# Rocco9999/2048_Q-Learning

Hardware: AMD Instinct MI355X
Metric: env_steps_per_sec (higher is better)
Workload: dtype u8

## Files before the change

2048_q-learning_amd/csrc/q2048_core.hpp:

```cpp
#pragma once
#include <stdint.h>
#include <math.h>

#if defined(__HIPCC__)
#define Q_HD __host__ __device__ __forceinline__
#else
#define Q_HD inline
#endif

#include "q2048_luts.inc"

namespace q2048 {

constexpr uint32_t kStreamStep = 0u, kStreamReset = 1u, kStreamOver = 2u;

struct Draws { uint32_t x0, x1, x2, x3; };

#ifndef Q2048_PHILOX_ROUNDS
#define Q2048_PHILOX_ROUNDS 10
#endif
Q_HD void philox_round(uint32_t& c0, uint32_t& c1, uint32_t& c2, uint32_t& c3, uint32_t k0, uint32_t k1) {
  const uint64_t p0 = (uint64_t)0xD2511F53u * c0;
  const uint64_t p1 = (uint64_t)0xCD9E8D57u * c2;
  const uint32_t n0 = (uint32_t)(p1 >> 32) ^ c1 ^ k0;
// ... 507 lines not shown

Q_HD uint64_t summary_fp(uint64_t hash) { return ((hash >> 48) & 0xffffull) | 1ull; }
struct SummaryHits { uint32_t ev, empty; };
Q_HD SummaryHits summary_decode(uint64_t word, uint64_t fp, uint32_t off) {
  uint32_t e = 0u, m = 0u;
#pragma unroll
  for (uint32_t r = 0; r < 4u; ++r) {
    const uint64_t f = (word >> (16u * r)) & 0xffffull;
    e |= (uint32_t)(f == 0ull) << r;
    m |= (uint32_t)(f == fp) << r;
  }
  return SummaryHits{(((e | m) | ((e | m) << 4)) >> (off & 3u)) & 15u, e};
}
Q_HD bool summary_pop(SummaryHits& h, uint32_t off, uint32_t& r, bool& absent) {
  if (h.ev == 0u) return false;
  r = (off + (uint32_t)__builtin_ctz(h.ev)) & 3u;
  absent = ((h.empty >> r) & 1u) != 0u;
  h.ev &= h.ev - 1u;
  return true;
}

Q_HD int argmax4(float q0, float q1, float q2, float q3) {
  int b = 0;
  float m = q0;
  if (q1 > m) { m = q1; b = 1; }
  if (q2 > m) { m = q2; b = 2; }
  if (q3 > m) { m = q3; b = 3; }
  return b;
}
Q_HD float max4(float q0, float q1, float q2, float q3) { return fmaxf(fmaxf(q0, q1), fmaxf(q2, q3)); }

Q_HD int eps_greedy(double eps, uint32_t x_eps, uint32_t x_act, float q0, float q1, float q2,
                    float q3, bool& explored) {
  explored = draw_uniform(x_eps) < eps;
  return explored ? draw_action(x_act) : argmax4(q0, q1, q2, q3);
}

Q_HD uint64_t eps_threshold(double eps) {
  if (!(eps > 0.0)) return 0ull;
  if (eps >= 1.0) return 1ull << 32;
  return (uint64_t)ceil(eps * 4294967296.0);
}
Q_HD bool draw_below(uint32_t x, uint64_t threshold) {
  return (threshold >> 32) != 0ull || x < (uint32_t)threshold;
}
Q_HD int eps_greedy_at(uint64_t threshold, uint32_t x_eps, uint32_t x_act, float q0, float q1, float q2,
                       float q3, bool& explored) {
  explored = draw_below(x_eps, threshold);
  return explored ? draw_action(x_act) : argmax4(q0, q1, q2, q3);
}

template <class BoardT>
Q_HD uint32_t legal_mask(const BoardT& b) {
  uint32_t m = 0;
#pragma unroll
  for (int a = 0; a < 4; ++a) {
    BoardT t = b;
    uint32_t score;
    m |= (uint32_t)move(t, a, score) << a;
  }
  return m;
}
Q_HD int play_action(uint32_t legal, float q0, float q1, float q2, float q3, uint64_t threshold, uint32_t x_eps,
                     uint32_t x_act, bool& explored) {
  legal &= 15u;
  const uint32_t n_legal = popc(legal);
  explored = n_legal != 0u && draw_below(x_eps, threshold);
  if (explored) {
    uint32_t k = draw_index(x_act, n_legal), m = legal;
#pragma unroll
    for (int j = 0; j < 3; ++j) { const bool drop = k != 0u; m &= drop ? m - 1u : m; k -= drop ? 1u : 0u; }
    return __builtin_ctz(m);
  }
  int best = 0;
  float top = 0.f;
  bool have = false;
  if (legal & 1u) { top = q0; have = true; }
  if ((legal & 2u) && (!have || q1 > top)) { top = q1; best = 1; have = true; }
  if ((legal & 4u) && (!have || q2 > top)) { top = q2; best = 2; have = true; }
  if ((legal & 8u) && (!have || q3 > top)) { top = q3; best = 3; }
  return best;
}

#if defined(__clang__)
#define Q2048_NO_CONTRACT _Pragma("clang fp contract(off)")
#else
#define Q2048_NO_CONTRACT
#endif
Q_HD double td_target(float reward, float max_q_next, bool done, double gamma) {
  Q2048_NO_CONTRACT
  const double bootstrap = gamma * (double)max_q_next;
  return (double)reward + bootstrap * (done ? 0.0 : 1.0);
}
Q_HD double td_fold(double q, double target, double lr) {
  Q2048_NO_CONTRACT
  const double step = lr * (target - q);
  return q + step;
}
Q_HD float td_value(float q_sa, float reward, float max_q_next, bool done, double lr,
                    double gamma) {
  return (float)td_fold((double)q_sa, td_target(reward, max_q_next, done, gamma), lr);
}

constexpr int kFoldMean = 0, kFoldMeanTrained = 1, kFoldSum = 2, kFoldMaxAbs = 3;
Q_HD void key_images(uint64_t k, uint64_t img[8]) {
  const uint64_t t = key_transpose(k), hk = key_flip_h(k), ht = key_flip_h(t);
  img[0] = k; img[1] = key_flip_v(t); img[2] = key_flip_v(hk); img[3] = ht;
  img[4] = hk; img[5] = t; img[6] = key_flip_v(k); img[7] = key_flip_v(ht);
}
Q_HD float fold_inv(uint32_t k) {
  return k == 1u ? 1.0f : k == 2u ? 0.5f : k == 3u ? (float)(1.0 / 3.0) : k == 4u ? 0.25f : k == 5u ? (float)(1.0 / 5.0)
       : k == 6u ? (float)(1.0 / 6.0) : k == 7u ? (float)(1.0 / 7.0) : 0.125f;
}
template <int FOLD>
Q_HD void fold_step(float& acc, uint32_t& n, float x) {
  Q2048_NO_CONTRACT
  if (FOLD == kFoldMeanTrained && x == 0.0f) return;
  if (n == 0u) acc = x;
  else if (FOLD == kFoldMaxAbs) acc = fabsf(x) > fabsf(acc) ? x : acc;
  else acc = acc + x;
  n += 1u;
}
template <int FOLD>
Q_HD float fold_finish(float acc, uint32_t n) {
  Q2048_NO_CONTRACT
  if (FOLD == kFoldMean || FOLD == kFoldMeanTrained) {
    const float inv = fold_inv(n);
    return n == 0u ? 0.0f : acc * inv;
  }
  return acc;
}
template <int FOLD, class Find>
Q_HD bool fold_orbit(uint64_t m, const float q[4], const Find& find, uint64_t& canon, float r[4]) {
  canon = canonical_key(m).key;
  uint64_t img[8];
  key_images(canon, img);
  float acc[4] = {0.0f, 0.0f, 0.0f, 0.0f};
  uint32_t n[4] = {0u, 0u, 0u, 0u};
  bool leader = false;
#pragma unroll
  for (int h = 0; h < 8; ++h) {
    bool repeat = false;
#pragma unroll
    for (int j = 0; j < h; ++j) repeat |= img[j] == img[h];
    if (repeat) continue;
    float v[4];
    if (img[h] == m) {
      leader = true;
      v[0] = q[0]; v[1] = q[1]; v[2] = q[2]; v[3] = q[3];
    } else {
      if (!find(img[h], v)) continue;
      if (!leader) return false;
    }
    const uint32_t g = canonical_key(img[h]).g;
#pragma unroll
    for (int a = 0; a < 4; ++a) {
      const int at = sym_action(g, a);
#pragma unroll
      for (int b = 0; b < 4; ++b)
        if (at == b) fold_step<FOLD>(acc[b], n[b], v[a]);
    }
  }
#pragma unroll
  for (int b = 0; b < 4; ++b) r[b] = fold_finish<FOLD>(acc[b], n[b]);
  return true;
}
// ... 37 lines not shown
```

2048_q-learning_amd/csrc/q2048_core5.hpp:

```cpp
#pragma once
#include "q2048_core.hpp"

namespace q2048 {

struct Board5 { uint32_t r[5]; };

constexpr uint32_t k5One = 0x01041041u;
constexpr uint32_t k5Low = k5One * 31u;
constexpr uint32_t k5High = k5One << 5;
constexpr uint32_t k5All = k5One * 63u;

Q_HD uint32_t nz5(uint32_t x) { return (x + k5Low) & k5High; }
Q_HD uint32_t z5(uint32_t x) { return ~(x + k5Low) & k5High; }
Q_HD uint32_t fill5(uint32_t m) { return m - (m >> 5); }
Q_HD uint32_t field5(uint32_t w, int c) { return (w >> (6 * c)) & 63u; }

Q_HD bool operator==(const Board5& a, const Board5& b) {
  uint32_t d = 0;
#pragma unroll
  for (int i = 0; i < 5; ++i) d |= a.r[i] ^ b.r[i];
  return d == 0;
}
Q_HD void clear(Board5& b) {
#pragma unroll
// ... 118 lines not shown
  for (int i = 1; i < 5; ++i) {
    const bool ge = k >= before[i];
    x = ge ? g[i] : x; base = ge ? before[i] : base; row += ge ? 1u : 0u;
  }
  const uint32_t skip = k - base;
#pragma unroll
  for (uint32_t j = 0; j < 4u; ++j) x = skip > j ? x & (x - 1u) : x;
  x &= 0u - x;
  const uint32_t w = x >> (draw_is_four(draw_val) ? 4u : 5u);
#pragma unroll
  for (int i = 0; i < 5; ++i) b.r[i] |= row == (uint32_t)i ? w : 0u;
  return n;
}
Q_HD void spawn(Board5& b, uint32_t draw_pos, uint32_t draw_val) { spawn_counted(b, true, draw_pos, draw_val); }

Q_HD bool game_over(const Board5& b) {
  uint32_t live = 0;
#pragma unroll
  for (int i = 0; i < 5; ++i) {
    live |= z5(b.r[i]);
    live |= z5(b.r[i] ^ (b.r[i] >> 6)) & (k5High >> 6);
    if (i < 4) live |= z5(b.r[i] ^ b.r[i + 1]);
  }
  return live == 0u;
}

Q_HD bool equal_neighbours_on_full(const Board5& b) {
  uint32_t acc = k5High;
#pragma unroll
  for (int i = 0; i < 5; ++i) {
    acc &= (b.r[i] ^ (b.r[i] >> 6)) + k5Low;
    if (i < 4) acc &= (b.r[i] ^ b.r[i + 1]) + k5Low;
  }
  return (acc & k5High) != k5High;
}

Q_HD bool spawn_then_over(Board5& b, bool valid, uint32_t draw_pos, uint32_t draw_val) {
  const uint32_t n = spawn_counted(b, valid, draw_pos, draw_val);
  const uint32_t left = n - ((valid && n != 0u) ? 1u : 0u);
  return left == 0u && !equal_neighbours_on_full(b);
}

Q_HD uint32_t fieldmax5(uint32_t a, uint32_t b) {
  const uint32_t m = fill5(((a | k5High) - b) & k5High);
  return bsel(m, a, b);
}
Q_HD uint32_t max_log2(const Board5& b) {
  uint32_t x = fieldmax5(fieldmax5(b.r[0], b.r[1]), fieldmax5(fieldmax5(b.r[2], b.r[3]), b.r[4]));
  uint32_t m = field5(x, 0);
#pragma unroll
  for (int c = 1; c < 5; ++c) { const uint32_t f = field5(x, c); m = f > m ? f : m; }
  return m;
}

struct Key5 { uint64_t k0, k1; };
Q_HD uint32_t pack_row5(uint32_t r) {
  return (r & 31u) | ((r >> 1) & (31u << 5)) | ((r >> 2) & (31u << 10)) | ((r >> 3) & (31u << 15)) |
         ((r >> 4) & (31u << 20));
}
Q_HD Key5 pack_key(const Board5& b) {
  const uint64_t p0 = pack_row5(b.r[0]), p1 = pack_row5(b.r[1]), p2 = pack_row5(b.r[2]),
                 p3 = pack_row5(b.r[3]), p4 = pack_row5(b.r[4]);
  return Key5{(p0 | (p1 << 25) | ((p2 & 0x1fffull) << 50)) | (1ull << 63),
              ((p2 >> 13) | (p3 << 12) | (p4 << 37)) | (1ull << 63)};
}
Q_HD uint32_t unpack_row5(uint32_t p) {
  return (p & 31u) | ((p & (31u << 5)) << 1) | ((p & (31u << 10)) << 2) | ((p & (31u << 15)) << 3) |
         ((p & (31u << 20)) << 4);
}
Q_HD Board5 unpack_key(const Key5& k) {
  const uint64_t a = k.k0 & ~(1ull << 63), c = k.k1 & ~(1ull << 63);
  Board5 b;
  b.r[0] = unpack_row5((uint32_t)(a & 0x1ffffffull));
  b.r[1] = unpack_row5((uint32_t)((a >> 25) & 0x1ffffffull));
  b.r[2] = unpack_row5((uint32_t)(((a >> 50) & 0x1fffull) | ((c & 0xfffull) << 13)));
  b.r[3] = unpack_row5((uint32_t)((c >> 12) & 0x1ffffffull));
  b.r[4] = unpack_row5((uint32_t)((c >> 37) & 0x1ffffffull));
  return b;
}

template <int N> struct Geo;
template <> struct Geo<4> {
  using BoardT = Board;
  struct Key { uint64_t k0; };
};
template <> struct Geo<5> {
  using BoardT = Board5;
  struct Key { uint64_t k0, k1; };
};
Q_HD bool key_eq(const Geo<4>::Key& a, const Geo<4>::Key& b) { return a.k0 == b.k0; }
Q_HD bool key_eq(const Geo<5>::Key& a, const Geo<5>::Key& b) { return a.k0 == b.k0 && a.k1 == b.k1; }
Q_HD uint64_t key_hash(const Geo<4>::Key& k) { return mix64(k.k0); }
Q_HD uint64_t key_hash(const Geo<5>::Key& k) { return mix64(k.k0 ^ (k.k1 * 0x9E3779B97F4A7C15ull)); }
template <class Key>
Q_HD uint64_t key_home(const Key& k, uint64_t mask) { return key_hash(k) & mask; }

template <class F>
Q_HD Geo<4>::Key state_key(const Board& b, uint64_t salt, const F& overflow) {
  bool ov;
  const uint64_t k = pack_key(b, ov) ^ salt;
  if (ov) overflow();
  return Geo<4>::Key{k != 0u ? k : 1u};
}
template <class F>
Q_HD Geo<5>::Key state_key(const Board5& b, uint64_t salt, const F&) {
  const Key5 k = pack_key(b);
  return Geo<5>::Key{k.k0 ^ (salt & 0x7fffffffffffffffull), k.k1 ^ (mix64(salt) & 0x3fffffffffffffffull)};
}
template <bool SYM, class BoardT, class F>
Q_HD auto state_key_as(const BoardT& b, uint64_t salt, uint32_t& g, const F& overflow) {
  if constexpr (SYM) {
    bool ov;
    const Canon c = canonical_key(pack_key(b, ov));
    if (ov) overflow();
    g = c.g;
    const uint64_t k = c.key ^ salt;
    return Geo<4>::Key{k != 0u ? k : 1u};
  } else {
    g = 0u;
    return state_key(b, salt, overflow);
  }
}

Q_HD Board5 board5_from_bytes(const uint8_t* p) {
  Board5 b;
#pragma unroll
  for (int i = 0; i < 5; ++i) {
    uint32_t w = 0;
#pragma unroll
    for (int c = 0; c < 5; ++c) w |= ((uint32_t)p[5 * i + c] & 31u) << (6 * c);
    b.r[i] = w;
  }
  return b;
}
Q_HD void board5_to_bytes(const Board5& b, uint8_t* p) {
#pragma unroll
  for (int i = 0; i < 5; ++i)
#pragma unroll
    for (int c = 0; c < 5; ++c) p[5 * i + c] = (uint8_t)(field5(b.r[i], c) & 31u);
}

}
```

2048_q-learning_amd/csrc/q2048_host.cpp:

```cpp
#include <algorithm>
#include <chrono>
#include <cstddef>
#include <cstdint>
#include <cstdlib>
#include <cstring>
#include <thread>
#include <unordered_map>
#include <vector>

#include "q2048_abi.hpp"
#include "q2048_core5.hpp"

namespace {
using namespace q2048;
using u64 = unsigned long long;

constexpr int kMaxAwait = 1 << 20;

static_assert(sizeof(q2048_aux) == 16 && sizeof(q2048_slot) == 32 && sizeof(q2048_episode) == 48, "ABI layout");
static_assert(sizeof(Aux) == sizeof(q2048_aux), "core/ABI aux mismatch");

inline void load_board(const uint8_t* boards, int64_t i, Board& b) { std::memcpy(&b, boards + 16 * i, 16); }
inline void load_board(const uint8_t* boards, int64_t i, Board5& b) { b = board5_from_bytes(boards + 25 * i); }
inline void store_board(uint8_t* boards, int64_t i, const Board& b) { std::memcpy(boards + 16 * i, &b, 16); }
inline void store_board(uint8_t* boards, int64_t i, const Board5& b) { board5_to_bytes(b, boards + 25 * i); }
inline Aux ld_aux(const q2048_aux* aux, int64_t i) {
  Words4 w;
  std::memcpy(&w, aux + i, 16);
  return words_to_aux(w);
}
inline void st_aux(q2048_aux* aux, int64_t i, const Aux& a) {
  const Words4 w = aux_to_words(a);
  std::memcpy(aux + i, &w, 16);
}
inline void status_or(uint32_t* status, uint32_t bits) { __atomic_fetch_or(status, bits, __ATOMIC_RELAXED); }

template <bool SYM, class BoardT>
inline auto state_key_as(const BoardT& b, u64 salt, uint32_t* status, uint32_t& g) {
  return q2048::state_key_as<SYM>(b, salt, g, [status] { status_or(status, Q2048_STATUS_TILE_OVERFLOW); });
}
template <class BoardT>
inline auto state_key(const BoardT& b, u64 salt, uint32_t* status) {
  uint32_t g;
  return state_key_as<false>(b, salt, status, g);
}
template <int N>
inline typename Geo<N>::Key state_key_sym(bool sym, const typename Geo<N>::BoardT& b, u64 salt, uint32_t* status, uint32_t& g) {
  if constexpr (N == 4) { if (sym) return state_key_as<true>(b, salt, status, g); }
  return state_key_as<false>(b, salt, status, g);
}

inline u64 ld_u64(const uint64_t* p) { return __atomic_load_n(p, __ATOMIC_ACQUIRE); }
inline float ld_f32(const float* p) {
  const uint32_t u = __atomic_load_n(reinterpret_cast<const uint32_t*>(p), __ATOMIC_RELAXED);
  return bits_f32(u);
}
inline void st_f32(float* p, float v) { __atomic_store_n(reinterpret_cast<uint32_t*>(p), f32_bits(v), __ATOMIC_RELAXED); }
inline Row ld_row(const q2048_slot* s) { return Row{ld_f32(&s->q[0]), ld_f32(&s->q[1]), ld_f32(&s->q[2]), ld_f32(&s->q[3])}; }

unsigned long long g_claim_timeouts = 0;
inline u64 await_second(const q2048_slot* s) {
  for (int spin = 0; spin < kMaxAwait; ++spin) {
    const u64 hi = ld_u64(&s->reserved);
    if (hi != 0ull) return hi;
    if ((spin & 1023) == 1023) std::this_thread::yield();
  }
  for (const auto give_up = std::chrono::steady_clock::now() + std::chrono::seconds(2); std::chrono::steady_clock::now() < give_up;) {
    std::this_thread::sleep_for(std::chrono::microseconds(50));
    const u64 hi = ld_u64(&s->reserved);
    if (hi != 0ull) return hi;
  }
  __atomic_fetch_add(&g_claim_timeouts, 1ull, __ATOMIC_RELAXED);
  return 0ull;
}
inline bool slot_is(const q2048_slot*, const Geo<4>::Key&) { return true; }
inline bool slot_is(const q2048_slot* s, const Geo<5>::Key& key) {
  u64 hi = ld_u64(&s->reserved);
  if (hi == 0ull) hi = await_second(s);
  return hi == key.k1;
}
inline void publish(q2048_slot*, const Geo<4>::Key&) {}
inline void publish(q2048_slot* s, const Geo<5>::Key& key) { __atomic_store_n(&s->reserved, key.k1, __ATOMIC_RELEASE); }

template <class Key>
inline int64_t probe_find(const q2048_slot* table, u64 mask, const Key& key, Row& row, uint32_t maxp = kRolloutProbe) {
  const Seq sq = seq_of(key_hash(key), mask);
  row = Row{0.f, 0.f, 0.f, 0.f};
  for (uint32_t p = 0, lim = probe_limit(mask, maxp); p < lim; ++p) {
    const u64 i = seq_slot(sq, p);
    const u64 k = ld_u64(&table[i].key);
    if (k == 0ull) return ~(int64_t)i;
    if (k == key.k0 && slot_is(&table[i], key)) { row = ld_row(&table[i]); return (int64_t)i; }
  }
  return kNoSlot;
}
inline int64_t probe_find_summary(const q2048_slot* table, const uint64_t* side, u64 mask, const Geo<5>::Key& key, Row& row,
                                  uint32_t maxp = kRolloutProbe) {
  const u64 hash = key_hash(key);
  const Seq sq = seq_of(hash, mask);
  const u64 fp = summary_fp(hash);
  row = Row{0.f, 0.f, 0.f, 0.f};
  for (uint32_t p = 0, lim = probe_limit(mask, maxp); p < lim; p += 4u) {
    const u64 line = (sq.line0 + (u64)(p >> 2)) & sq.lmask;
    SummaryHits hits = summary_decode(ld_u64(&side[line]), fp, sq.off);
    uint32_t r;
    bool absent;
    while (summary_pop(hits, sq.off, r, absent)) {
      const u64 i = (line << 2) | (u64)r;
      if (absent) return ~(int64_t)i;
      if (ld_u64(&table[i].key) == key.k0 && ld_u64(&table[i].reserved) == key.k1) { row = ld_row(&table[i]); return (int64_t)i; }
    }
  }
  return kNoSlot;
}
inline int64_t probe_find_summary(const q2048_slot* table, const uint64_t*, u64 mask, const Geo<4>::Key& key, Row& row) {
  return probe_find(table, mask, key, row);
}
template <class Key>
inline int64_t probe_insert(q2048_slot* table, u64 mask, const Key& key, u64 start, bool& inserted,
                            uint32_t maxp = kRolloutProbe) {
  const Seq sq = seq_of(key_hash(key), mask);
  inserted = false;
  u64 i = start & mask;
  for (uint32_t p = seq_pos(sq, i), lim = probe_limit(mask, maxp); p < lim; i = seq_slot(sq, ++p)) {
    uint64_t k = ld_u64(&table[i].key);
    if (k == 0ull) {
      uint64_t expect = 0ull;
      if (__atomic_compare_exchange_n(&table[i].key, &expect, (uint64_t)key.k0, false, __ATOMIC_ACQ_REL, __ATOMIC_ACQUIRE)) {
        publish(&table[i], key);
        inserted = true;
// ... 268 lines not shown
  if (!boards || !actions || !status) return Q2048_ERR_NULL;
  if (!aligned16(boards) || !aligned16(row_cache)) return Q2048_ERR_ALIGN;
  if (!(eps >= 0.0 && eps <= 1.0)) return Q2048_ERR_RANGE;
  if (B == 0) return Q2048_OK;
  const u64 mask = (1ull << cap_log2) - 1ull;
  if (n == 4) q_choose_impl_n<4>(table, mask, boards, B, eps, seed, env_id0, ctr, flags, actions, status, draw_eps, draw_act, row_cache);
  else q_choose_impl_n<5>(table, mask, boards, B, eps, seed, env_id0, ctr, flags, actions, status, draw_eps, draw_act, row_cache);
  return Q2048_OK;
}

template <int N>
void q_update_impl_n(q2048_slot* table, u64 mask, const uint8_t* s, const uint8_t* actions, const float* reward,
                     const uint8_t* s2, const uint8_t* done, int64_t B, double lr, double gamma, uint64_t env_id0,
                     uint32_t flags, int64_t* stats_i, uint32_t* status, void* cache) {
  const int T = threads_for(B);
  std::vector<Stats> parts((size_t)T);
  Stats* sp = parts.data();
  const bool cas = (flags & Q2048_FLAG_TD_CAS) != 0, create = (flags & Q2048_FLAG_NO_NEW_ROWS) == 0;
  const int used = parallel_ranges(B, [=](int64_t lo, int64_t hi, int t) {
    Stats& st = sp[t];
    TdCounters tdc;
    for (int64_t i = lo; i < hi; ++i) {
      const int act = actions[i];
      if (act > 3) { status_or(status, Q2048_STATUS_BAD_ACTION); continue; }
      typename Geo<N>::BoardT b_s, b_n;
      load_board(s, i, b_s);
      load_board(s2, i, b_n);
      const u64 salt = (flags & Q2048_FLAG_INDEPENDENT) ? lane_salt(env_id0 + (uint64_t)i) : 0ull;
      const auto key_s = state_key(b_s, salt, status);
      const auto key_n = state_key(b_n, salt, status);
      Row rs, rn;
      bool ins_s = false, ins_n = false;
      int64_t slot = kNoSlot;
      if (!cache_get<N>(cache, i, table, mask, key_s, rs, slot, !create)) slot = find_or_create(table, mask, key_s, rs, ins_s, create);
      rn = rs;
      const bool same = key_eq(key_n, key_s);
      int64_t slot_n = slot;
      if (!same) slot_n = find_or_create(table, mask, key_n, rn, ins_n, create);
      st.i[Q2048_ST_INSERTS] += (uint64_t)ins_s + (uint64_t)ins_n;
      const float max_next = max4(rn.q0, rn.q1, rn.q2, rn.q3);
      if (slot >= 0) {
        const float nq = td_update(&table[slot], act, row_get(rs, act), reward[i], max_next, done[i] != 0, lr, gamma, cas, tdc);
        if (same) row_set(rn, act, nq);
      } else {
        st.i[Q2048_ST_DROPS] += 1;
        if (create) status_or(status, Q2048_STATUS_TABLE_FULL);
        else if (same) row_set(rn, act, td_value(row_get(rs, act), reward[i], max_next, done[i] != 0, lr, gamma));
      }
      cache_put<N>(cache, i, table, mask, key_n, rn, slot_n, !create);
    }
    st.i[Q2048_ST_CAS_RETRY] += tdc.retries;
    st.i[Q2048_ST_CAS_FALLBACK] += tdc.fallbacks;
  });
  stats_merge(parts, used, stats_i, nullptr);
}

template <int N>
void q_lookup_impl_n(const q2048_slot* table, u64 mask, const uint8_t* boards, int64_t B, uint64_t env_id0,
                     uint32_t flags, float* q_out, uint8_t* found, uint32_t* status) {
  const bool sym = (flags & Q2048_FLAG_SYMMETRIC) != 0;
  parallel_ranges(B, [=](int64_t lo, int64_t hi, int) {
    for (int64_t i = lo; i < hi; ++i) {
      typename Geo<N>::BoardT b;
      load_board(boards, i, b);
      const uint64_t id = (flags & Q2048_FLAG_SINGLE_ENV) ? env_id0 : env_id0 + (uint64_t)i;
      const u64 salt = (flags & Q2048_FLAG_INDEPENDENT) ? lane_salt(id) : 0ull;
      Row r;
      uint32_t g;
      const int64_t slot = probe_find(table, mask, state_key_sym<N>(sym, b, salt, status, g), r, kMaxProbe);
      if (sym) r = row_env(r, g);
      q_out[4 * i] = r.q0; q_out[4 * i + 1] = r.q1; q_out[4 * i + 2] = r.q2; q_out[4 * i + 3] = r.q3;
      if (found != nullptr) found[i] = slot >= 0;
    }
  });
}

constexpr int kGroup = 16;
template <int N>
void fused_rollout_n(uint8_t* boards, q2048_aux* aux, q2048_slot* table, u64 mask, int64_t B, int steps, double eps,
                     double lr, double gamma, uint64_t seed, uint64_t env_id0, uint32_t ctr0, uint32_t flags,
                     int64_t* stats_i, double* stats_f, uint32_t* status, q2048_episode* log, int64_t log_cap,
                     uint64_t* log_count, void* cache, const uint64_t* side) {
  using BoardT = typename Geo<N>::BoardT;
  using Key = typename Geo<N>::Key;
  struct Lane {
    BoardT b; Aux a; Key key_s, key_n; Row q; int64_t slot_s; u64 salt; uint64_t id; double reward_sum;
    StepOut o; int act; bool explored, same; DrawPrep prep;
    uint32_t g_s, g_n;
  };
  const uint64_t eps_t = eps_threshold(eps);
  const ImageLuts lut{&g_lut_image};
  const int env = env_bits(flags);
  const bool play_only = (flags & Q2048_FLAG_PLAY_ONLY) != 0, no_learn = (flags & Q2048_FLAG_NO_LEARN) != 0;
  const bool learns = !play_only && !no_learn, frozen = (flags & Q2048_FLAG_NO_NEW_ROWS) != 0;
  const bool creates = learns && !frozen, cas = (flags & Q2048_FLAG_TD_CAS) != 0;
  const bool sym = N == 4 && !play_only && (flags & Q2048_FLAG_SYMMETRIC) != 0;
  const bool summary = N == 5 && learns && frozen && (flags & Q2048_FLAG_LINE_SUMMARY) != 0 && side != nullptr;
  const int T = threads_for(B);
  std::vector<Stats> parts((size_t)T);
  Stats* sp = parts.data();
  const int used = parallel_ranges(B, [=](int64_t lo, int64_t hi, int tid) {
    auto find = [=](const Key& key, Row& row) {
      return summary ? probe_find_summary(table, side, mask, key, row) : probe_find(table, mask, key, row);
    };
    Stats& st = sp[tid];
    TdCounters tdc;
    bool any_drop = false;
    Lane lane[kGroup];
    for (int64_t g0 = lo; g0 < hi; g0 += kGroup) {
      const int n = (int)(hi - g0 < kGroup ? hi - g0 : kGroup);
      for (int l = 0; l < n; ++l) {
        Lane& L = lane[l];
        const int64_t i = g0 + l;
        L.id = env_id0 + (uint64_t)i;
        L.salt = (flags & Q2048_FLAG_INDEPENDENT) ? lane_salt(L.id) : 0ull;
        load_board(boards, i, L.b);
        L.a = ld_aux(aux, i);
        L.key_s = state_key_sym<N>(sym, L.b, L.salt, status, L.g_s);
        L.q = Row{0.f, 0.f, 0.f, 0.f};
        L.slot_s = play_only ? kNoSlot : find(L.key_s, L.q);
        if (frozen && learns && L.slot_s < 0) visit_get<N>(cache, i, table, mask, L.key_s, L.q);
        L.reward_sum = 0.0;
        L.prep = draws_prepare(seed, L.id, kStreamStep);
      }
      for (int t = 0; t < steps; ++t) {
        for (int l = 0; l < n; ++l) {
          Lane& L = lane[l];
          const Draws x = draws_at(L.prep, ctr0 + (uint32_t)t);
          Draws y{0u, 0u, 0u, 0u};
          if (env & kEnvDqn) y = draws(seed, L.id, ctr0 + (uint32_t)t, kStreamOver);
          const Row qe = sym ? row_env(L.q, L.g_s) : L.q;
          L.act = eps_greedy_at(eps_t, x.x0, x.x1, qe.q0, qe.q1, qe.q2, qe.q3, L.explored);
          L.o = env_step_any(env, L.b, L.a, L.act, x.x2, x.x3, y.x0, y.x1, lut);
          L.key_n = state_key_sym<N>(sym, L.b, L.salt, status, L.g_n);
          L.same = key_eq(L.key_n, L.key_s);
          if (!L.same && !play_only) __builtin_prefetch(&table[key_hash(L.key_n) & mask], 1, 1);
        }
        for (int l = 0; l < n; ++l) {
          Lane& L = lane[l];
          const StepOut& o = L.o;
          const int act = sym ? sym_action(L.g_s, L.act) : L.act;
          bool ins_s = false, ins_n = false;
          if (L.slot_s < 0 && L.slot_s != kNoSlot && creates) L.slot_s = probe_insert(table, mask, L.key_s, (u64)~L.slot_s, ins_s);
          Row qn = L.q;
          int64_t slot_n = L.slot_s;
          if (!L.same) {
            if (play_only) { qn = Row{0.f, 0.f, 0.f, 0.f}; slot_n = kNoSlot; }
            else if (creates) slot_n = find_or_create(table, mask, L.key_n, qn, ins_n);
            else slot_n = find(L.key_n, qn);
          }
          const float max_next = max4(qn.q0, qn.q1, qn.q2, qn.q3);
          const bool updated = L.slot_s >= 0;
          float nq = 0.f;
          if (updated) {
            if (no_learn) nq = td_value(row_get(L.q, act), o.reward, max_next, o.done != 0, lr, gamma);
            else nq = td_update(&table[L.slot_s], act, row_get(L.q, act), o.reward, max_next, o.done != 0, lr, gamma, cas, tdc);
          } else if (frozen && learns) {
            nq = td_value(row_get(L.q, act), o.reward, max_next, o.done != 0, lr, gamma);
          }
          st.i[Q2048_ST_VALID] += o.valid != 0;
          st.i[Q2048_ST_EXPLORE] += L.explored;
          st.i[Q2048_ST_INSERTS] += (uint64_t)ins_s + (uint64_t)ins_n;
          if (!updated && learns) { st.i[Q2048_ST_DROPS] += 1; any_drop = any_drop || !frozen; }
          L.reward_sum += (double)o.reward;
          if (o.done) {
            st.i[Q2048_ST_EPISODES] += 1;
            st.episode(L.a, o.max_log2);
            if (log != nullptr) {
              const uint64_t at = __atomic_fetch_add(log_count, (uint64_t)1, __ATOMIC_RELAXED);
              if ((int64_t)at < log_cap) {
                Row ql = L.q;
                if ((updated || (frozen && learns)) && !no_learn) row_set(ql, act, nq);
                q2048_episode rec;
                if (sym) ql = row_env(ql, L.g_s);
                rec.env_id = L.id; rec.episode = L.a.episode; rec.action = (uint8_t)L.act;
                rec.max_log2 = o.max_log2; rec.steps_lo = (uint16_t)(ctr0 + (uint32_t)t);
                rec.reward = o.reward; rec.total_return = L.a.ep_return; rec.score = L.a.score;
                rec.q[0] = ql.q0; rec.q[1] = ql.q1; rec.q[2] = ql.q2; rec.q[3] = ql.q3;
                rec.reserved = 0u;
                log[at] = rec;
              }
            }
            begin_episode(L.b, L.a, seed, L.id, (env & kEnvResetShaping) != 0);
            L.key_s = state_key_sym<N>(sym, L.b, L.salt, status, L.g_s);
            L.q = Row{0.f, 0.f, 0.f, 0.f};
            L.slot_s = play_only ? kNoSlot : find(L.key_s, L.q);
          } else if (L.same) {
            if ((updated || (frozen && learns)) && !no_learn) row_set(L.q, act, nq);
            else if (!updated) L.slot_s = kNoSlot;
          } else {
            L.key_s = L.key_n; L.slot_s = slot_n; L.q = qn; L.g_s = L.g_n;
          }
        }
      }
      for (int l = 0; l < n; ++l) {
        st.i[Q2048_ST_STEPS] += (uint64_t)steps;
        st.f[Q2048_SF_REWARD] += lane[l].reward_sum;
        store_board(boards, g0 + l, lane[l].b);
        st_aux(aux, g0 + l, lane[l].a);
        if (!play_only) visit_put<N>(cache, g0 + l, table, mask, lane[l].key_s, lane[l].q, frozen && learns && lane[l].slot_s < 0);
      }
    }
    st.i[Q2048_ST_CAS_RETRY] += tdc.retries;
    st.i[Q2048_ST_CAS_FALLBACK] += tdc.fallbacks;
    if (any_drop) status_or(status, Q2048_STATUS_TABLE_FULL);
  });
  stats_merge(parts, used, stats_i, stats_f);
}

template <int N>
void play_rollout_n(uint8_t* boards, q2048_aux* aux, const q2048_slot* table, u64 mask, int64_t B, int steps, double eps,
                    uint64_t seed, uint64_t env_id0, uint32_t ctr0, uint32_t flags, int64_t* stats_i, double* stats_f,
                    uint32_t* status) {
  const uint64_t eps_t = eps_threshold(eps);
  const ImageLuts lut{&g_lut_image};
  const int env = env_bits(flags);
  const bool sym = (flags & Q2048_FLAG_SYMMETRIC) != 0;
  const int T = threads_for(B);
  std::vector<Stats> parts((size_t)T);
  Stats* sp = parts.data();
  const int used = parallel_ranges(B, [=](int64_t lo, int64_t hi, int tid) {
    Stats& st = sp[tid];
    for (int64_t i = lo; i < hi; ++i) {
      const uint64_t id = env_id0 + (uint64_t)i;
      const u64 salt = (flags & Q2048_FLAG_INDEPENDENT) ? lane_salt(id) : 0ull;
      typename Geo<N>::BoardT b;
      load_board(boards, i, b);
      Aux a = ld_aux(aux, i);
      const DrawPrep prep = draws_prepare(seed, id, kStreamStep);
      double reward_sum = 0.0;
      for (int t = 0; t < steps; ++t) {
        const Draws x = draws_at(prep, ctr0 + (uint32_t)t);
        Draws y{0u, 0u, 0u, 0u};
        if (env & kEnvDqn) y = draws(seed, id, ctr0 + (uint32_t)t, kStreamOver);
        Row q;
        uint32_t g;
        probe_find(table, mask, state_key_sym<N>(sym, b, salt, status, g), q, kMaxProbe);
        if (sym) q = row_env(q, g);
        bool explored;
        const int act = play_action(legal_mask(b), q.q0, q.q1, q.q2, q.q3, eps_t, x.x0, x.x1, explored);
        const StepOut o = env_step_any(env, b, a, act, x.x2, x.x3, y.x0, y.x1, lut);
        st.i[Q2048_ST_VALID] += o.valid != 0;
        st.i[Q2048_ST_EXPLORE] += explored;
        reward_sum += (double)o.reward;
        if (o.done) {
          st.i[Q2048_ST_EPISODES] += 1;
          st.episode(a, o.max_log2);
          begin_episode(b, a, seed, id, (env & kEnvResetShaping) != 0);
        }
      }
      st.i[Q2048_ST_STEPS] += (uint64_t)steps;
      st.f[Q2048_SF_REWARD] += reward_sum;
      store_board(boards, i, b);
      st_aux(aux, i, a);
    }
  });
  stats_merge(parts, used, stats_i, stats_f);
}

template <int N>
void det_rollout_n(uint8_t* boards, q2048_aux* aux, q2048_slot* table, u64 mask, int64_t B, int64_t steps, double eps,
                   double lr, double gamma, uint64_t seed, uint64_t env_id0, uint32_t ctr0, uint32_t flags,
                   int64_t* stats_i, double* stats_f, uint32_t* status, void* row_cache) {
  const int env = env_bits(flags);
  const bool create = (flags & Q2048_FLAG_NO_NEW_ROWS) == 0;
  void* const cache = create ? nullptr : row_cache;
  std::vector<int64_t> cell((size_t)B);
  std::vector<double> target((size_t)B);
  int64_t* cp = cell.data();
  double* tp = target.data();
  const int T = threads_for(B);
  for (int64_t t = 0; t < steps; ++t) {
    std::vector<Stats> parts((size_t)T);
    Stats* sp = parts.data();
    const uint32_t ctr = ctr0 + (uint32_t)t;
    const int used = parallel_ranges(B, [=](int64_t lo, int64_t hi, int tid) {
      Stats& st = sp[tid];
      for (int64_t i = lo; i < hi; ++i) {
        const uint64_t id = env_id0 + (uint64_t)i;
        const u64 salt = (flags & Q2048_FLAG_INDEPENDENT) ? lane_salt(id) : 0ull;
        typename Geo<N>::BoardT b;
// ... 764 lines not shown
```

2048_q-learning_amd/csrc/q2048_kernels.hip:

```cpp
#include <hip/hip_runtime.h>
#include <stddef.h>
#include <stdint.h>

#include <cstdio>
#include <cstdlib>
#include <cstring>
#include <ctime>
#include <condition_variable>
#include <deque>
#include <functional>
#include <map>
#include <mutex>
#include <thread>
#include <vector>

#include "q2048_abi.hpp"
#include "q2048_core5.hpp"

#ifdef Q2048_EXPERIMENTS
#define Q2048_XBITS(flags, shift, mask) (((flags) >> (shift)) & (mask))
#else
#define Q2048_XBITS(flags, shift, mask) 0u
#endif

// ... 793 lines not shown
    } else {
      const u64 salt = (flags & Q2048_FLAG_INDEPENDENT) ? lane_salt(env_id0 + (uint64_t)i) : 0ull;
      const auto key_s = state_key(b_s, salt, status);
      const auto key_n = state_key(b_n, salt, status);
      const bool same = key_eq(key_n, key_s);
      Row rs;
      int64_t slot = kNoSlot;
      if (cache == nullptr || !cache_get(cache, i, key_s, cache_tag(table, mask), rs, slot, frozen)) {
        slot = probe_find(table, mask, key_s, rs, ins_s);
        if (slot < 0 && slot != kNoSlot && !frozen) slot = probe_insert(table, mask, key_s, (u64)~slot, ins_s);
      }
      Row rn = rs;
      int64_t slot_n = slot;
      Claim claim{0ull, 0ull, false};
      if (!same) {
        slot_n = probe_find(table, mask, key_n, rn, ins_n);
        if constexpr (!frozen) slot_n = claim_issue(table, mask, slot_n, key_n, claim, ins_n);
      }
      const float max_next = max4(rn.q0, rn.q1, rn.q2, rn.q3);
      if (slot >= 0) {
        const float nq = td_update(&table[slot], act, row_get(rs, act), rew, max_next, is_done,
                                   lr, gamma, tdc, td_mode_of(flags));
        if (same) row_set(rn, act, nq);
      } else {
        dropped = true;
        if (!frozen) atomicOr(status, Q2048_STATUS_TABLE_FULL);
        else if (same)
          row_set(rn, act, td_value(row_get(rs, act), rew, max_next, is_done, lr, gamma));
      }
      bool ins_c = false;
      slot_n = claim_resolve(table, mask, key_n, claim, slot_n, ins_c);
      ins_n = ins_n || ins_c;
      if (cache != nullptr) cache_put(cache, i, key_n, cache_tag(table, mask), rn, slot_n, frozen);
    }
    const uint32_t n_ins = wave_count(ins_n) + wave_count(ins_s), n_drop = wave_count(dropped);
    if (tdc.retries) atomicAdd(&bs.i[Q2048_ST_CAS_RETRY], (u64)tdc.retries);
    if (tdc.fallbacks) atomicAdd(&bs.i[Q2048_ST_CAS_FALLBACK], (u64)tdc.fallbacks);
    if (wave_leader()) {
      if (n_ins) atomicAdd(&bs.i[Q2048_ST_INSERTS], (u64)n_ins);
      if (n_drop) atomicAdd(&bs.i[Q2048_ST_DROPS], (u64)n_drop);
    }
  }
  stats_flush(bs, stats_i, nullptr);
}

#ifdef Q2048_FUSED_MIN_WAVES
#define Q2048_FUSED_WAVES(N) Q2048_FUSED_MIN_WAVES
#else
#define Q2048_FUSED_WAVES(N) ((N) == 4 ? 6 : 5)
#endif
constexpr int kModeLearn = 0, kModeCas = 1, kModeEval = 2, kModeFrozen = 4, kModeSummary = 8;
constexpr int kModeSym = 16;
constexpr int kFusedBlockBig = 512, kFusedBlockSmall = kBlock;
constexpr int64_t kFusedBigBatch = 786432;
#ifdef Q2048_EXPERIMENTS
__device__ unsigned long long* g_timeline;
#define Q2048_STAMP(k) do { if (g_timeline != nullptr && threadIdx.x == 0) {                       \
    g_timeline[(size_t)blockIdx.x * 8 + (k)] = wall_clock64();                                     \
    if ((k) == 0) {                                                                                \
      g_timeline[(size_t)blockIdx.x * 8 + 4] = (unsigned)__builtin_amdgcn_s_getreg((31 << 11) | 4);   \
      g_timeline[(size_t)blockIdx.x * 8 + 5] = (unsigned)__builtin_amdgcn_s_getreg((31 << 11) | 20);  \
    } } } while (0)
#else
#define Q2048_STAMP(k) do { } while (0)
#endif
__device__ const LutImage g_lut_image = Q2048_LUT_IMAGE;
template <int N, int ENV, int MODE, int BLOCK>
__global__ __launch_bounds__(BLOCK, Q2048_FUSED_WAVES(N)) void k_fused_rollout(
    uint8_t* boards, q2048_aux* aux, q2048_slot* table, u64 mask, int64_t B, int steps, double eps,
    double lr, double gamma, uint64_t seed, uint64_t env_id0, uint32_t ctr0, uint32_t flags,
    int64_t* stats_i, double* stats_f, uint32_t* status, q2048_episode* log, int64_t log_cap,
    u64* log_count, void* row_cache, u64* mirror, uint32_t* ticket, const u64* side) {
  RowCache<N>* const cache = static_cast<RowCache<N>*>(row_cache);
  __shared__ BlockStats bs;
  __shared__ Stage<N, BLOCK / 64> st;
  __shared__ LutImage lut_lds;
  static_assert(BLOCK >= kLutImageDoubles, "one double of the image per thread");
  Q2048_STAMP(0);
  if (threadIdx.x < kLutImageDoubles)
    reinterpret_cast<double*>(&lut_lds)[threadIdx.x] = reinterpret_cast<const double*>(&g_lut_image)[threadIdx.x];
  stats_clear(bs);
  const ImageLuts lut{&lut_lds};
  const int64_t i = (int64_t)blockIdx.x * BLOCK + threadIdx.x;
  auto b = load_board(boards, i, B, st);
  if (i < B) {
    const uint64_t id = env_id0 + (uint64_t)i;
    const u64 salt = (flags & Q2048_FLAG_INDEPENDENT) ? lane_salt(id) : 0ull;
    constexpr bool play_only = (ENV & kEnvPlayOnly) != 0;
    constexpr bool no_learn = (MODE & ~kModeSym) == kModeEval;
    constexpr bool sym = (MODE & kModeSym) != 0;
    static_assert(!sym || (N == 4 && !play_only), "symmetry folding: 4x4 learners, evaluators and frozen tables");
    constexpr bool frozen = (MODE & kModeFrozen) != 0;
    constexpr bool summary = (MODE & kModeSummary) != 0;
#ifdef Q2048_EXPERIMENTS
    const uint32_t td_mode = no_learn ? (uint32_t)kTdNone : td_mode_of(flags);
    const bool x_noclaim = ((flags >> 12) & 1u) || play_only || no_learn || frozen, x_noprobe = ((flags >> 13) & 1u) || play_only;
    const bool may_defer = td_mode == kTdStorePlain && !((flags >> 14) & 1u);
    const int max_cas = ((flags >> 16) & 0xffu) ? (int)((flags >> 16) & 0xffu) : kMaxCas;
#else
    constexpr uint32_t td_mode = no_learn ? kTdNone : ((MODE & kModeCas) ? kTdCas : kTdStorePlain);
    constexpr bool x_noclaim = play_only || no_learn || frozen, x_noprobe = play_only;
    constexpr bool may_defer = td_mode == kTdStorePlain;
    constexpr int max_cas = kMaxCas;
#endif
    Aux a = ld_aux(aux, i);
    uint32_t g_s;
    auto key_s = state_key_as<sym>(b, salt, status, g_s);
    Row q{0.f, 0.f, 0.f, 0.f};
    bool made0 = false;
    int64_t slot_s = kNoSlot;
    if (!play_only && (cache == nullptr || !cache_get(cache, i, key_s, cache_tag(table, mask), q, slot_s, frozen)))
      slot_s = probe_find_as<summary>(table, side, mask, key_s, q, made0);
    Claim claim{0ull, 0ull, false};
    uint32_t n_valid = 0, n_explore = 0, n_done = 0, n_insert = wave_count(made0), n_drop = 0;
    uint32_t pend = 0;
    TdCounters tdc{0u, 0u};
    double reward_sum = 0.0;
    const DrawPrep prep_x = draws_prepare(seed, id, kStreamStep);
    const uint64_t eps_t = eps_threshold(eps);

    for (int t = 0; t < steps; ++t) {
      const Draws x = draws_at(prep_x, ctr0 + (uint32_t)t);
      Draws y{0u, 0u, 0u, 0u};
      if constexpr ((ENV & kEnvDqn) != 0) y = draws(seed, id, ctr0 + (uint32_t)t, kStreamOver);
      bool explored;
      Row qe = q;
      if constexpr (sym) qe = row_env(q, g_s);
      const int act_env = eps_greedy_at(eps_t, x.x0, x.x1, qe.q0, qe.q1, qe.q2, qe.q3, explored);
      const StepOut o = env_step_profile<ENV>(b, a, act_env, x.x2, x.x3, y.x0, y.x1, lut);
      const int act = sym ? sym_action(g_s, act_env) : act_env;
      uint32_t g_n;
      const auto key_n = state_key_as<sym>(b, salt, status, g_n);
      const bool same = key_eq(key_n, key_s);
      bool ins_s = false, ins_n = false;
      slot_s = claim_resolve(table, mask, key_s, claim, slot_s, ins_s);
      if (slot_s < 0 && slot_s != kNoSlot && !x_noclaim)
        slot_s = probe_insert(table, mask, key_s, (u64)~slot_s, ins_s);
      Row qn = q;
      int64_t slot_n = slot_s;
      if (!same) {
        if (x_noprobe) { qn = Row{0.f, 0.f, 0.f, 0.f}; slot_n = ~(int64_t)key_home(key_n, mask); }
        else slot_n = probe_find_as<summary>(table, side, mask, key_n, qn, ins_n);
      }
      const float max_next = max4(qn.q0, qn.q1, qn.q2, qn.q3);
      float nq = 0.f;
      const bool updated = slot_s >= 0;
      if (updated) {
        if (same && !o.done && may_defer) {
          nq = td_value(row_get(q, act), o.reward, max_next, false, lr, gamma);
          pend |= 1u << act;
        } else {
          nq = td_update(&table[slot_s], act, row_get(q, act), o.reward, max_next, o.done != 0, lr,
                         gamma, tdc, td_mode, max_cas);
          pend &= ~(1u << act);
          if (pend) flush_pending(&table[slot_s], q, pend);
        }
      } else if (frozen) {
        nq = td_value(row_get(q, act), o.reward, max_next, o.done != 0, lr, gamma);
      }
      if (o.done) {
        if (!same && slot_n < 0 && slot_n != kNoSlot && !x_noclaim)
          probe_insert(table, mask, key_n, (u64)~slot_n, ins_n);
        episode_stats(bs, a, o.max_log2);
        if (log != nullptr) {
          const u64 at = atomicAdd(log_count, 1ull);
          if ((int64_t)at < log_cap) {
            Row ql = q;
            if ((updated || frozen) && !no_learn) row_set(ql, act, nq);
            if constexpr (sym) ql = row_env(ql, g_s);
            q2048_episode rec;
            rec.env_id = id; rec.episode = a.episode; rec.action = (uint8_t)act_env;
            rec.max_log2 = o.max_log2; rec.steps_lo = (uint16_t)(ctr0 + (uint32_t)t);
            rec.reward = o.reward; rec.total_return = a.ep_return; rec.score = a.score;
            rec.q[0] = ql.q0; rec.q[1] = ql.q1; rec.q[2] = ql.q2; rec.q[3] = ql.q3;
            rec.reserved = 0u;
            log[at] = rec;
          }
        }
        begin_episode(b, a, seed, id, (ENV & kEnvResetShaping) != 0);
        key_s = state_key_as<sym>(b, salt, status, g_s);
        bool made = false;
        q = Row{0.f, 0.f, 0.f, 0.f};
        slot_s = play_only ? kNoSlot : probe_find_as<summary>(table, side, mask, key_s, q, made);
        ins_n = ins_n || made;
      } else if (same) {
        if ((updated || frozen) && !no_learn) row_set(q, act, nq);
        else if (!updated) slot_s = kNoSlot;
      } else {
        key_s = key_n; slot_s = slot_n; q = qn; g_s = g_n;
        if (!x_noclaim) {
          bool made = false;
          slot_s = claim_issue(table, mask, slot_s, key_s, claim, made);
          ins_n = ins_n || made;
        }
      }
      n_valid += wave_count(o.valid != 0);
      n_explore += wave_count(explored);
      n_insert += wave_count(ins_s) + wave_count(ins_n);
      n_drop += wave_count(!updated && !play_only && !no_learn);
      n_done += wave_count(o.done != 0);
      reward_sum += (double)o.reward;
      if (t == 0) Q2048_STAMP(1);
    }
    Q2048_STAMP(2);
    if (pend && slot_s >= 0) flush_pending(&table[slot_s], q, pend);
    bool ins_last = false;
    slot_s = claim_resolve(table, mask, key_s, claim, slot_s, ins_last);
    n_insert += wave_count(ins_last);
    st_aux(aux, i, a);
    if (!play_only && cache != nullptr) cache_put(cache, i, key_s, cache_tag(table, mask), q, slot_s, frozen);

    if (n_drop && !frozen) atomicOr(status, Q2048_STATUS_TABLE_FULL);
    if (tdc.retries) atomicAdd(&bs.i[Q2048_ST_CAS_RETRY], (u64)tdc.retries);
    if (tdc.fallbacks) atomicAdd(&bs.i[Q2048_ST_CAS_FALLBACK], (u64)tdc.fallbacks);
    atomicAdd(&bs.f[Q2048_SF_REWARD], reward_sum);
    const uint32_t n_active = wave_count(true);
    if (wave_leader()) {
      atomicAdd(&bs.i[Q2048_ST_STEPS], (u64)n_active * (u64)steps);
      atomicAdd(&bs.i[Q2048_ST_VALID], (u64)n_valid);
      atomicAdd(&bs.i[Q2048_ST_EXPLORE], (u64)n_explore);
      atomicAdd(&bs.i[Q2048_ST_EPISODES], (u64)n_done);
      atomicAdd(&bs.i[Q2048_ST_INSERTS], (u64)n_insert);
      atomicAdd(&bs.i[Q2048_ST_DROPS], (u64)n_drop);
    }
  }
  store_board(boards, i, B, b, st);
  if (mirror == nullptr) {
    stats_flush(bs, stats_i, stats_f);
  } else {
    stats_flush_acked(bs, stats_i, stats_f);
    stats_mirror(stats_i, stats_f, mirror, ticket);
  }
  Q2048_STAMP(3);
}

template <int N, int ENV, bool SYM = false>
__global__ __launch_bounds__(kBlock) void k_play_rollout(
    uint8_t* boards, q2048_aux* aux, const q2048_slot* table, u64 mask, int64_t B, int steps, double eps,
    uint64_t seed, uint64_t env_id0, uint32_t ctr0, uint32_t flags, int64_t* stats_i, double* stats_f,
    uint32_t* status) {
  __shared__ BlockStats bs;
  __shared__ Stage<N> st;
  __shared__ LutImage lut_lds;
  static_assert(kBlock >= kLutImageDoubles, "one double of the image per thread");
  if (threadIdx.x < kLutImageDoubles)
    reinterpret_cast<double*>(&lut_lds)[threadIdx.x] = reinterpret_cast<const double*>(&g_lut_image)[threadIdx.x];
  stats_clear(bs);
  const ImageLuts lut{&lut_lds};
  const int64_t i = (int64_t)blockIdx.x * kBlock + threadIdx.x;
  auto b = load_board(boards, i, B, st);
  if (i < B) {
    const uint64_t id = env_id0 + (uint64_t)i;
    const u64 salt = (flags & Q2048_FLAG_INDEPENDENT) ? lane_salt(id) : 0ull;
    Aux a = ld_aux(aux, i);
    uint32_t n_valid = 0, n_explore = 0, n_done = 0;
    double reward_sum = 0.0;
    const DrawPrep prep_x = draws_prepare(seed, id, kStreamStep);
    const uint64_t eps_t = eps_threshold(eps);
    for (int t = 0; t < steps; ++t) {
      const Draws x = draws_at(prep_x, ctr0 + (uint32_t)t);
      Draws y{0u, 0u, 0u, 0u};
      if constexpr ((ENV & kEnvDqn) != 0) y = draws(seed, id, ctr0 + (uint32_t)t, kStreamOver);
      Row q;
      bool made;
      uint32_t g;
      probe_find(table, mask, state_key_as<SYM>(b, salt, status, g), q, made, kMaxProbe);
      if constexpr (SYM) q = row_env(q, g);
      bool explored;
      const int act = play_action(legal_mask(b), q.q0, q.q1, q.q2, q.q3, eps_t, x.x0, x.x1, explored);
      const StepOut o = env_step_profile<ENV>(b, a, act, x.x2, x.x3, y.x0, y.x1, lut);
      if (o.done) {
        episode_stats(bs, a, o.max_log2);
        begin_episode(b, a, seed, id, (ENV & kEnvResetShaping) != 0);
      }
      n_valid += wave_count(o.valid != 0);
      n_explore += wave_count(explored);
      n_done += wave_count(o.done != 0);
      reward_sum += (double)o.reward;
    }
    st_aux(aux, i, a);
    atomicAdd(&bs.f[Q2048_SF_REWARD], reward_sum);
    const uint32_t n_active = wave_count(true);
    if (wave_leader()) {
      atomicAdd(&bs.i[Q2048_ST_STEPS], (u64)n_active * (u64)steps);
      atomicAdd(&bs.i[Q2048_ST_VALID], (u64)n_valid);
      atomicAdd(&bs.i[Q2048_ST_EXPLORE], (u64)n_explore);
      atomicAdd(&bs.i[Q2048_ST_EPISODES], (u64)n_done);
    }
  }
  store_board(boards, i, B, b, st);
  stats_flush(bs, stats_i, stats_f);
}

constexpr int kDetHashShift = 44, kDetHashBits = 16;
constexpr u64 kDetSlotMask = (1ull << kDetHashShift) - 1ull;
constexpr u64 kDetDrop = 1ull << 62, kDetDone = 1ull << 63;
constexpr uint32_t kNoCarry = 0xffffffffu;
__device__ __forceinline__ Row ld_row(const q2048_slot* s) {
  const u32x4 v = ld16_agent(&s->q[0]);
  return Row{bits_f32(v.x), bits_f32(v.y), bits_f32(v.z), bits_f32(v.w)};
}
template <int N, int ENV, bool VISITS>
__device__ __forceinline__ void det_phase1_body(
    uint8_t* boards, q2048_aux* aux, q2048_slot* table, u64 mask, int64_t B, double eps, double gamma,
    uint64_t seed, uint64_t env_id0, uint32_t ctr, uint32_t flags, u64* group_out, double* target_out,
    uint32_t* carry, int use_carry, StatStripe* stat_stripes, uint32_t* gs0, int n_gs, uint32_t* status,
    RowCache<N>* cache, double lr) {
  __shared__ BlockStats bs;
  __shared__ Stage<N> st;
// ... 2146 lines not shown
```

Baseline: 22.61 billion.

## Step 4x4 boards in packed nibble form with bit-sliced slide and merge

Adds a packed board type for 4x4 games that stores tiles as 4-bit nibbles in two 32-bit words plus an overflow mask. The move, spawn, game-over and max-tile operations are implemented directly on the nibble layout, with the transpose done by bit shuffles. Boards fall back to the byte layout when a tile exceeds the nibble range. The training kernel and host path convert to this representation at load and back at store. The goal is fewer registers and ALU ops per step, at the cost of a per-step wide-tile check and extra pack/unpack work at the kernel edges.

```diff
diff --git a/2048_q-learning_amd/csrc/q2048_core.hpp b/2048_q-learning_amd/csrc/q2048_core.hpp
--- a/2048_q-learning_amd/csrc/q2048_core.hpp
+++ b/2048_q-learning_amd/csrc/q2048_core.hpp
@@ -613,6 +613,145 @@
   return best;
 }
 
+struct PBoard { uint32_t lo, hi, x; };
+
+Q_HD bool operator==(const PBoard& a, const PBoard& b) { return ((a.lo ^ b.lo) | (a.hi ^ b.hi) | (a.x ^ b.x)) == 0; }
+Q_HD void clear(PBoard& b) { b = PBoard{0u, 0u, 0u}; }
+Q_HD uint64_t packed_key(const PBoard& b) { return (uint64_t)b.lo | ((uint64_t)b.hi << 32); }
+Q_HD uint64_t pack_key(const PBoard& b, bool& overflow) { overflow = b.x != 0u; return packed_key(b); }
+
+Q_HD PBoard pack_board(const Board& b) {
+  return PBoard{pack_row(b.r0) | (pack_row(b.r1) << 16), pack_row(b.r2) | (pack_row(b.r3) << 16),
+                movemask((b.r0 << 3) & 0x80808080u) | (movemask((b.r1 << 3) & 0x80808080u) << 4) |
+                (movemask((b.r2 << 3) & 0x80808080u) << 8) | (movemask((b.r3 << 3) & 0x80808080u) << 12)};
+}
+Q_HD uint32_t unpack_row_x(uint32_t k, uint32_t x4) {
+  return unpack_row(k) | ((((x4 & 0xfu) * 0x00204081u) & 0x01010101u) << 4);
+}
+Q_HD Board unpack_board(const PBoard& b) {
+  return Board{unpack_row_x(b.lo, b.x), unpack_row_x(b.lo >> 16, b.x >> 4), unpack_row_x(b.hi, b.x >> 8),
+               unpack_row_x(b.hi >> 16, b.x >> 12)};
+}
+
+Q_HD uint32_t nz8(uint32_t x) { x |= x << 1; x |= x << 2; return x & 0x88888888u; }
+Q_HD uint32_t z8(uint32_t x) { x |= x << 1; x |= x << 2; return ~x & 0x88888888u; }
+Q_HD uint32_t fill8(uint32_t m) { return (m << 1) - (m >> 3); }
+Q_HD bool packed_wide(const PBoard& b) {
+  uint32_t l = b.lo & (b.lo >> 1), h = b.hi & (b.hi >> 1);
+  l &= l >> 2; h &= h >> 2;
+  return (((l | h) & 0x11111111u) | b.x) != 0u;
+}
+
+Q_HD PBoard transpose(const PBoard& b) {
+  const uint32_t l = (b.lo & 0xf0f00f0fu) | ((b.lo & 0x0000f0f0u) << 12) | ((b.lo >> 12) & 0x0000f0f0u);
+  const uint32_t h = (b.hi & 0xf0f00f0fu) | ((b.hi & 0x0000f0f0u) << 12) | ((b.hi >> 12) & 0x0000f0f0u);
+  return PBoard{(l & 0x00ff00ffu) | ((h & 0x00ff00ffu) << 8), ((l >> 8) & 0x00ff00ffu) | (h & 0xff00ff00u), b.x};
+}
+
+Q_HD uint32_t pow2_sum_n(uint32_t v) {
+  return (((1u << (v & 15u)) & ~1u) + ((1u << ((v >> 4) & 15u)) & ~1u)) +
+         (((1u << ((v >> 8) & 15u)) & ~1u) + ((1u << ((v >> 12) & 15u)) & ~1u));
+}
+
+Q_HD uint32_t slide_lines_n(uint32_t& c0, uint32_t& c1, uint32_t& c2, uint32_t& c3) {
+  uint32_t z;
+#pragma unroll
+  for (int rep = 0; rep < 3; ++rep) {
+    z = fill8(z8(c0) & 0x8888u);
+    c0 = bsel(z, c1, c0); c1 = bsel(z, c2, c1); c2 = bsel(z, c3, c2); c3 &= ~z;
+  }
+#pragma unroll
+  for (int rep = 0; rep < 2; ++rep) {
+    z = fill8(z8(c1) & 0x8888u);
+    c1 = bsel(z, c2, c1); c2 = bsel(z, c3, c2); c3 &= ~z;
+  }
+  z = fill8(z8(c2) & 0x8888u);
+  c2 = bsel(z, c3, c2); c3 &= ~z;
+  uint32_t e = z8(c0 ^ c1) & nz8(c0);
+  uint32_t m = fill8(e);
+  c0 += e >> 3;
+  const uint32_t s_a = c0 & m;
+  c1 = bsel(m, c2, c1); c2 = bsel(m, c3, c2); c3 &= ~m;
+  e = z8(c1 ^ c2) & nz8(c1);
+  m = fill8(e);
+  c1 += e >> 3;
+  const uint32_t s_b = c1 & m;
+  c2 = bsel(m, c3, c2); c3 &= ~m;
+  e = z8(c2 ^ c3) & nz8(c2);
+  m = fill8(e);
+  c2 += e >> 3;
+  c3 &= ~m;
+  const uint32_t s_c = c2 & m;
+  return pow2_sum_n(s_a | s_c) + pow2_sum_n(s_b);
+}
+
+Q_HD uint32_t rot16(uint32_t x) { return (x << 16) | (x >> 16); }
+Q_HD bool move(PBoard& b, int action, uint32_t& score) {
+  const bool horiz = (action & 1) == 0, rev = (action & 2) != 0;
+  const PBoard t = transpose(b);
+  const uint32_t pl = horiz ? t.lo : b.lo, ph = horiz ? t.hi : b.hi;
+  const uint32_t wl = rev ? rot16(ph) : pl, wh = rev ? rot16(pl) : ph;
+  uint32_t c0 = wl & 0xffffu, c1 = wl >> 16, c2 = wh & 0xffffu, c3 = wh >> 16;
+  score = slide_lines_n(c0, c1, c2, c3);
+  const uint32_t nl = c0 | (c1 << 16), nh = c2 | (c3 << 16);
+  const bool moved = ((nl ^ wl) | (nh ^ wh)) != 0;
+  const PBoard q{rev ? rot16(nh) : nl, rev ? rot16(nl) : nh, b.x};
+  const PBoard qt = transpose(q);
+  b.lo = horiz ? qt.lo : q.lo; b.hi = horiz ? qt.hi : q.hi;
+  return moved;
+}
+
+Q_HD uint32_t movemask_n(uint32_t m8) {
+  uint32_t v = m8 >> 3;
+  v = (v | (v >> 3)) & 0x03030303u;
+  v = (v | (v >> 6)) & 0x000f000fu;
+  return (v | (v >> 12)) & 0xffu;
+}
+Q_HD uint32_t empty_mask(const PBoard& b) { return movemask_n(z8(b.lo)) | (movemask_n(z8(b.hi)) << 8); }
+
+Q_HD void spawn(PBoard& b, uint32_t draw_pos, uint32_t draw_val) {
+  const uint32_t zl = z8(b.lo), zh = z8(b.hi), nl = popc(zl), n = nl + popc(zh);
+  if (n == 0u) return;
+  uint32_t k = draw_index(draw_pos, n), c, sh = 0u;
+  const bool up = k >= nl;
+  k -= up ? nl : 0u;
+  uint32_t m = up ? zh : zl;
+  bool ge;
+  c = popc(m & 0xffffu); ge = k >= c; k -= ge ? c : 0u; sh += ge ? 16u : 0u; m >>= ge ? 16u : 0u;
+  c = popc(m & 0xffu);   ge = k >= c; k -= ge ? c : 0u; sh += ge ? 8u : 0u;  m >>= ge ? 8u : 0u;
+  c = (m >> 3) & 1u;     ge = k >= c; sh += ge ? 4u : 0u;
+  const uint32_t w = (draw_is_four(draw_val) ? 2u : 1u) << sh;
+  b.lo |= up ? 0u : w; b.hi |= up ? w : 0u;
+}
+
+Q_HD bool game_over(const PBoard& b) {
+  const uint32_t empties = z8(b.lo) | z8(b.hi);
+  const uint32_t mid = (b.lo >> 16) | (b.hi << 16);
+  const uint32_t vert = z8(b.lo ^ mid) | (z8(b.hi ^ (b.hi >> 16)) & 0x00008888u);
+  const uint32_t horz = (z8(b.lo ^ (b.lo >> 4)) | z8(b.hi ^ (b.hi >> 4))) & 0x08880888u;
+  return (empties | vert | horz) == 0u;
+}
+
+Q_HD uint32_t max_log2(const PBoard& b) {
+  uint32_t x = bytemax(bytemax(b.lo & 0x0f0f0f0fu, (b.lo >> 4) & 0x0f0f0f0fu),
+                       bytemax(b.hi & 0x0f0f0f0fu, (b.hi >> 4) & 0x0f0f0f0fu));
+  x = bytemax(x, x >> 16);
+  x = bytemax(x, x >> 8);
+  return x & 0xffu;
+}
+
+template <int ENV, class LutT = ConstLuts>
+Q_HD StepOut env_step_profile(PBoard& b, Aux& a, int action, uint32_t x_pos, uint32_t x_val, uint32_t y_pos,
+                              uint32_t y_val, const LutT& lut = LutT()) {
+  if (packed_wide(b)) {
+    Board w = unpack_board(b);
+    const StepOut o = env_step_profile<ENV, Board, LutT>(w, a, action, x_pos, x_val, y_pos, y_val, lut);
+    b = pack_board(w);
+    return o;
+  }
+  return env_step_profile<ENV, PBoard, LutT>(b, a, action, x_pos, x_val, y_pos, y_val, lut);
+}
+
 #if defined(__clang__)
 #define Q2048_NO_CONTRACT _Pragma("clang fp contract(off)")
 #else
diff --git a/2048_q-learning_amd/csrc/q2048_core5.hpp b/2048_q-learning_amd/csrc/q2048_core5.hpp
--- a/2048_q-learning_amd/csrc/q2048_core5.hpp
+++ b/2048_q-learning_amd/csrc/q2048_core5.hpp
@@ -224,12 +224,18 @@
 template <int N> struct Geo;
 template <> struct Geo<4> {
   using BoardT = Board;
+  using StepT = PBoard;
   struct Key { uint64_t k0; };
 };
 template <> struct Geo<5> {
   using BoardT = Board5;
+  using StepT = Board5;
   struct Key { uint64_t k0, k1; };
 };
+Q_HD PBoard to_step(const Board& b) { return pack_board(b); }
+Q_HD const Board5& to_step(const Board5& b) { return b; }
+Q_HD Board from_step(const PBoard& b) { return unpack_board(b); }
+Q_HD const Board5& from_step(const Board5& b) { return b; }
 Q_HD bool key_eq(const Geo<4>::Key& a, const Geo<4>::Key& b) { return a.k0 == b.k0; }
 Q_HD bool key_eq(const Geo<5>::Key& a, const Geo<5>::Key& b) { return a.k0 == b.k0 && a.k1 == b.k1; }
 Q_HD uint64_t key_hash(const Geo<4>::Key& k) { return mix64(k.k0); }
@@ -239,6 +245,13 @@
 
 template <class F>
 Q_HD Geo<4>::Key state_key(const Board& b, uint64_t salt, const F& overflow) {
+  bool ov;
+  const uint64_t k = pack_key(b, ov) ^ salt;
+  if (ov) overflow();
+  return Geo<4>::Key{k != 0u ? k : 1u};
+}
+template <class F>
+Q_HD Geo<4>::Key state_key(const PBoard& b, uint64_t salt, const F& overflow) {
   bool ov;
   const uint64_t k = pack_key(b, ov) ^ salt;
   if (ov) overflow();
diff --git a/2048_q-learning_amd/csrc/q2048_host.cpp b/2048_q-learning_amd/csrc/q2048_host.cpp
--- a/2048_q-learning_amd/csrc/q2048_host.cpp
+++ b/2048_q-learning_amd/csrc/q2048_host.cpp
@@ -44,8 +44,8 @@
   uint32_t g;
   return state_key_as<false>(b, salt, status, g);
 }
-template <int N>
-inline typename Geo<N>::Key state_key_sym(bool sym, const typename Geo<N>::BoardT& b, u64 salt, uint32_t* status, uint32_t& g) {
+template <int N, class BoardT>
+inline typename Geo<N>::Key state_key_sym(bool sym, const BoardT& b, u64 salt, uint32_t* status, uint32_t& g) {
   if constexpr (N == 4) { if (sym) return state_key_as<true>(b, salt, status, g); }
   return state_key_as<false>(b, salt, status, g);
 }
@@ -480,9 +480,10 @@
                      int64_t* stats_i, double* stats_f, uint32_t* status, q2048_episode* log, int64_t log_cap,
                      uint64_t* log_count, void* cache, const uint64_t* side) {
   using BoardT = typename Geo<N>::BoardT;
+  using StepT = typename Geo<N>::StepT;
   using Key = typename Geo<N>::Key;
   struct Lane {
-    BoardT b; Aux a; Key key_s, key_n; Row q; int64_t slot_s; u64 salt; uint64_t id; double reward_sum;
+    StepT b; Aux a; Key key_s, key_n; Row q; int64_t slot_s; u64 salt; uint64_t id; double reward_sum;
     StepOut o; int act; bool explored, same; DrawPrep prep;
     uint32_t g_s, g_n;
   };
@@ -512,7 +513,9 @@
         const int64_t i = g0 + l;
         L.id = env_id0 + (uint64_t)i;
         L.salt = (flags & Q2048_FLAG_INDEPENDENT) ? lane_salt(L.id) : 0ull;
-        load_board(boards, i, L.b);
+        BoardT b_in;
+        load_board(boards, i, b_in);
+        L.b = to_step(b_in);
         L.a = ld_aux(aux, i);
         L.key_s = state_key_sym<N>(sym, L.b, L.salt, status, L.g_s);
         L.q = Row{0.f, 0.f, 0.f, 0.f};
@@ -594,7 +597,7 @@
       for (int l = 0; l < n; ++l) {
         st.i[Q2048_ST_STEPS] += (uint64_t)steps;
         st.f[Q2048_SF_REWARD] += lane[l].reward_sum;
-        store_board(boards, g0 + l, lane[l].b);
+        store_board(boards, g0 + l, from_step(lane[l].b));
         st_aux(aux, g0 + l, lane[l].a);
         if (!play_only) visit_put<N>(cache, g0 + l, table, mask, lane[l].key_s, lane[l].q, frozen && learns && lane[l].slot_s < 0);
       }
diff --git a/2048_q-learning_amd/csrc/q2048_kernels.hip b/2048_q-learning_amd/csrc/q2048_kernels.hip
--- a/2048_q-learning_amd/csrc/q2048_kernels.hip
+++ b/2048_q-learning_amd/csrc/q2048_kernels.hip
@@ -899,7 +899,7 @@
   stats_clear(bs);
   const ImageLuts lut{&lut_lds};
   const int64_t i = (int64_t)blockIdx.x * BLOCK + threadIdx.x;
-  auto b = load_board(boards, i, B, st);
+  auto b = to_step(load_board(boards, i, B, st));
   if (i < B) {
     const uint64_t id = env_id0 + (uint64_t)i;
     const u64 salt = (flags & Q2048_FLAG_INDEPENDENT) ? lane_salt(id) : 0ull;
@@ -1041,7 +1041,7 @@
       atomicAdd(&bs.i[Q2048_ST_DROPS], (u64)n_drop);
     }
   }
-  store_board(boards, i, B, b, st);
+  store_board(boards, i, B, from_step(b), st);
   if (mirror == nullptr) {
     stats_flush(bs, stats_i, stats_f);
   } else {
```

Result: no change. 22.41 billion (-0.9%).
